# bdaiinstitute/vlfm

Hardware: AMD Instinct MI355X
Metric: env-steps/s (VLM+value-map update), 640x480 RGB-D (higher is better)
Workload: dtype f16 ViT-g (f32 accumulate) + f32 Q-Former (split-f16, 22-bit); f32 confidence + f64 value maps; 1 GPU; configs[1] step x resident envs: BLIP-2 ITC + ValueMap+ObstacleMap+sort_waypoints; envs_per_gpu=256, global_envs=256, map=1000x1000 @ 20 px/m, parallelism=env-sharded x1, tuned_gemms=True, vit_gemm=hip:fc1, attention=hip

## Files before the change

### include/vlfm_amd.h

```cpp
#ifndef VLFM_AMD_H
#define VLFM_AMD_H

#include <stddef.h>
#include <stdint.h>

#ifdef __cplusplus
extern "C" {
#endif

typedef enum {
    VLFM_OK = 0,
    VLFM_ERR_INVALID = -1,
    VLFM_ERR_OUTSIDE_MAP = -2,
    VLFM_ERR_INDEX = -3,
    VLFM_ERR_HIP = -4,
    VLFM_ERR_CAPACITY = -5
} vlfm_status;

enum { VLFM_FUSE_DEFAULT = 0, VLFM_FUSE_REPLACE = 1, VLFM_FUSE_EQUAL_WEIGHTING = 2 };

const char* vlfm_last_error(void);
int vlfm_abi_version(void);

int vlfm_profile_enable(int on);
// ... 134 lines not shown
                        const int32_t* d_text_index, int n_prompts, float* d_out, void* stream);

int vlfm_layernorm_bias_f16(const void* d_x, const float* d_channel_bias, const void* d_gamma, const void* d_beta,
                            void* d_y, int rows, int dim, float eps, void* stream);

int vlfm_vit_attention_f16(const void* d_qkv, void* d_out, int batch, int tokens, int heads, int head_dim, float scale,
                           void* stream);

int vlfm_gemm_f16_nt(const void* d_x, const void* d_w, const void* d_bias, void* d_c, int m, int n, int k, int epilogue,
                     void* stream);

int vlfm_gemm_f16_pair_f32_nt(const void* d_x, const void* d_w_pair, const void* d_bias_f32, void* d_out, int m, int n_out, int k,
                              void* stream);

int vlfm_qformer_cross_attention_f32(const void* d_q, const void* d_kv_blocks, void* d_out, int batch, int tokens, int queries,
                                     int heads, int k_block0, int v_block0, int m_total, float scale, void* stream);

int vlfm_gemm_f16_tile_order(int m, int n, int group_m, int* out, int capacity_pairs);
int vlfm_gemm_f16_work_items(int m, int n, int grid, int* out, int capacity_pairs);

int vlfm_split_f32_to_f16_pair(const float* d_src, void* d_hi, void* d_lo, long long count, int* d_overflow, void* stream);
int vlfm_gemm_f32_nt(const float* d_x, const float* d_w, const float* d_bias, const float* d_residual, float* d_c, int m, int n,
                     int k, int activation, int precision, const void* d_w_hi, const void* d_w_lo, int* d_overflow, void* stream);


int vlfm_layernorm_rows_f32(const float* d_x, const float* d_gamma, const float* d_beta, float* d_out, int batch, int height,
                            int width, int channels, int window, float eps, void* stream);
int vlfm_window_reverse_add_f32(float* d_x, const float* d_windows, int batch, int height, int width, int channels, int window,
                                void* stream);
int vlfm_dwconv3x3_nhwc_f32(const float* d_x, const float* d_w9c, const float* d_bias, float* d_out, int batch, int height, int width,
                            int channels, void* stream);
int vlfm_window_attention_f32(const float* d_qkv, const float* d_bias_t, float* d_out, long long windows, int tokens, int heads,
                              float scale, void* stream);
int vlfm_layernorm_rows_shifted_f32(const float* d_x, const float* d_gamma, const float* d_beta, float* d_out, int batch, int height,
                                    int width, int channels, int window, float eps, int shift, int pad_zero, void* stream);
int vlfm_window_reverse_add_shifted_f32(float* d_x, const float* d_windows, int batch, int height, int width, int channels, int window,
                                        int shift, void* stream);
int vlfm_window_attention_masked_f32(const float* d_qkv, const float* d_bias_t, const float* d_mask_t, int windows_per_image, float* d_out,
                                     long long windows, int tokens, int heads, float scale, void* stream);

int vlfm_maxpool2x2_nhwc_f16(const void* d_x, void* d_out, int batch, int height, int width, int channels, void* stream);
int vlfm_conv_nhwc_tile(int pixels, int cin, int cout, int ksize, int* tile_pixels, int* tile_channels);
int vlfm_conv_nhwc_f16(const void* d_x, const void* d_w, const void* d_bias, void* d_out, const void* d_zero, int batch,
                       int height, int width, int cin, int cout, int ksize, int stride, int x_pix_stride,
                       int out_pix_stride, int act, void* stream);

// ... 188 lines not shown
```

### vlfm_amd/_lib.py

```python
from __future__ import annotations

import ctypes
import os
import subprocess
from typing import Optional

_HERE = os.path.dirname(os.path.abspath(__file__))
LIB_PATH = os.path.join(_HERE, "libvlfm_amd.so")
SOURCES = ["value_map.hip", "depth_ingest.hip", "depth_holes.hip", "obstacle_map.hip", "vlm_ops.hip", "vit_attention.hip", "qformer_attention.hip", "detect_ops.hip", "object_cloud.hip", "gemm_f16.hip", "gemm_f32.hip", "conv_nhwc.hip", "sam_ops.hip", "map_render.hip", "jpeg_codec.hip", "jpeg_entropy.hip", "jpeg_decode.hip", "world_render.hip", "host.cpp"]

VLFM_OK = 0
VLFM_ERR_INVALID = -1
VLFM_ERR_OUTSIDE_MAP = -2
VLFM_ERR_INDEX = -3
VLFM_ERR_HIP = -4
VLFM_ERR_CAPACITY = -5

FUSION_TYPES = {"default": 0, "replace": 1, "equal_weighting": 2}


class VmPose(ctypes.Structure):
    _fields_ = [("inv_affine", ctypes.c_double * 6), ("row0", ctypes.c_int32), ("col0", ctypes.c_int32),
                ("env", ctypes.c_int32), ("reserved", ctypes.c_int32)]

# ... 80 lines not shown
        L.vlfm_profile_read.argtypes = [ctypes.c_char_p, ctypes.POINTER(cd), ctypes.POINTER(ci)]
        L.vlfm_value_map_pose_params.argtypes = [vp, vp, vp, ci, ci, ci, ci, vp, ctypes.POINTER(ci)]
        L.vlfm_cone_template_host.argtypes = [cd, cd, ci, cd, vp, ci, vp, ci, ctypes.POINTER(ci)]
        L.vlfm_tan_table_host.argtypes = [cd, ci, vp]
        L.vlfm_disc_rows_host.argtypes = [ci, vp]
        L.vlfm_cone_template_build.argtypes = [vp, vp, ci, ci, vp, vp, vp]
        L.vlfm_depth_ingest_batched.argtypes = [vp, ci, ci, ci, vp, vp, vp, ci, ci, vp, vp, vp, vp, vp]
        L.vlfm_selftest_div_exact.argtypes = [vp, ci, cd, vp, vp]
        L.vlfm_hole_scratch_bytes.argtypes = [ci, ci, ci, ci, ci]
        L.vlfm_hole_scratch_bytes.restype = ctypes.c_size_t
        L.vlfm_fill_small_holes_batched.argtypes = [vp, vp, ci, ci, ci, cd, vp, ctypes.c_size_t, ci, ci, vp, vp, vp, vp,
                                                    ci, vp, vp]
        L.vlfm_depth_scatter_holes_batched.argtypes = [vp, ci, ci, ci, vp, vp, vp, vp, ci, ci, vp, vp, vp]
        L.vlfm_fill_small_holes_rig_batched.argtypes = [vp, vp, ci, ci, ci, cd, vp, ctypes.c_size_t, ci, ci, vp, vp, vp, vp,
                                                        ci, vp, vp, ci, vp]
        L.vlfm_depth_scatter_holes_rig_batched.argtypes = [vp, ci, ci, ci, vp, vp, vp, vp, ci, ci, vp, vp, vp, vp]
        L.vlfm_layernorm_bias_f16.argtypes = [vp, vp, vp, vp, vp, ci, ci, ctypes.c_float, vp]
        L.vlfm_vit_attention_f16.argtypes = [vp, vp, ci, ci, ci, ci, ctypes.c_float, vp]
        L.vlfm_gemm_f16_nt.argtypes = [vp, vp, vp, vp, ci, ci, ci, ci, vp]
        L.vlfm_gemm_f16_pair_f32_nt.argtypes = [vp, vp, vp, vp, ci, ci, ci, vp]
        L.vlfm_qformer_cross_attention_f32.argtypes = [vp, vp, vp, ci, ci, ci, ci, ci, ci, ci, ctypes.c_float, vp]
        L.vlfm_gemm_f32_nt.argtypes = [vp, vp, vp, vp, vp, ci, ci, ci, ci, ci, vp, vp, vp, vp]
        L.vlfm_split_f32_to_f16_pair.argtypes = [vp, vp, vp, ctypes.c_longlong, vp, vp]
        L.vlfm_layernorm_rows_f32.argtypes = [vp, vp, vp, vp, ci, ci, ci, ci, ci, ctypes.c_float, vp]
        L.vlfm_window_reverse_add_f32.argtypes = [vp, vp, ci, ci, ci, ci, ci, vp]
        L.vlfm_dwconv3x3_nhwc_f32.argtypes = [vp, vp, vp, vp, ci, ci, ci, ci, vp]
        L.vlfm_window_attention_f32.argtypes = [vp, vp, vp, ctypes.c_longlong, ci, ci, ctypes.c_float, vp]
        L.vlfm_layernorm_rows_shifted_f32.argtypes = [vp, vp, vp, vp, ci, ci, ci, ci, ci, ctypes.c_float, ci, ci, vp]
        L.vlfm_window_reverse_add_shifted_f32.argtypes = [vp, vp, ci, ci, ci, ci, ci, ci, vp]
        L.vlfm_window_attention_masked_f32.argtypes = [vp, vp, vp, ci, vp, ctypes.c_longlong, ci, ci, ctypes.c_float, vp]
        L.vlfm_maxpool2x2_nhwc_f16.argtypes = [vp, vp, ci, ci, ci, ci, vp]
        L.vlfm_conv_nhwc_tile.argtypes = [ci, ci, ci, ci, ctypes.POINTER(ci), ctypes.POINTER(ci)]
        L.vlfm_conv_nhwc_f16.argtypes = [vp, vp, vp, vp, vp, ci, ci, ci, ci, ci, ci, ci, ci, ci, ci, vp]
        L.vlfm_value_map_update_fused_batched.argtypes = [vp, ci, vp, vp, vp, ci, vp, vp, ci, vp, vp, ci, ci, ci, cd, cd,
                                                          ci, ci, vp, vp, vp, vp, vp]
        L.vlfm_value_map_update_rig_batched.argtypes = [vp, ci, vp, vp, vp, ci, ci, ci, vp, vp, vp, ci, ci, ci, ci, ci, vp, vp,
                                                        vp, vp]
        L.vlfm_value_map_sort_waypoints_batched.argtypes = [vp, ci, ci, vp, ci, ci, vp, ci, vp, vp]
        L.vlfm_resample_coeffs_host.argtypes = [ci, ci, vp, vp, ci, ctypes.POINTER(ci)]
        L.vlfm_resample_coeffs_filter_host.argtypes = [ci, ci, ci, vp, vp, ci, ctypes.POINTER(ci)]
        L.vlfm_preprocess_sam_batched.argtypes = [vp, ci, ci, ci, ci, ci, vp, vp, ci, vp, vp, ci, vp, vp, ci, vp, vp, vp]
        L.vlfm_preprocess_rgb_batched.argtypes = [vp, ci, ci, ci, ci, vp, vp, ci, vp, vp, ci, vp, vp, vp, vp, ci, ci, vp]
        L.vlfm_itc_head_batched.argtypes = [vp, ci, ci, ci, vp, vp, vp]
        L.vlfm_itc_head_multi.argtypes = [vp, ci, ci, ci, vp, ci, vp, ci, vp, vp]
        cf = ctypes.c_float
        L.vlfm_resize_area_tab_host.argtypes = [ci, ci, vp, vp, vp, ci]
# ... 111 lines not shown
```

### vlfm_amd/csrc/gemm_f32.hip

```cpp
#include <hip/hip_runtime.h>
#include <stdint.h>
#include <stdlib.h>

#include "../../include/vlfm_amd.h"
#include "profile.h"
#include "status.h"

namespace vlfm {
namespace g32 {

typedef float floatx4 __attribute__((ext_vector_type(4)));
typedef float floatx16 __attribute__((ext_vector_type(16)));
typedef _Float16 half8 __attribute__((ext_vector_type(8)));
typedef _Float16 half4 __attribute__((ext_vector_type(4)));

constexpr int TB = 128;
constexpr int TK = 32;
constexpr int ROWB = TK * 4;
constexpr int OPER = TB * ROWB;
constexpr int BUF = 2 * OPER;
constexpr int EPI_ROW = 272;
constexpr int EPI_WAVE = 64 * EPI_ROW;
constexpr int LDS_EXACT = 4 * EPI_WAVE > 2 * BUF ? 4 * EPI_WAVE : 2 * BUF;

enum { ACT_NONE = 0, ACT_RELU = 1, ACT_GELU = 2 };

struct Args {
    const float* x;
    const float* w;
    const float* bias;
    const float* residual;
    float* c;
    int M, N, K;
    int tiles_m, tiles_n;
    int* overflow;
    const _Float16* w_hi;
    const _Float16* w_lo;
};

__device__ inline float gelu_erf(float v) {
    const float u = fabsf(v);
    float q = 2.834908400e-06f;
    q = fmaf(q, u, -3.937762449e-05f);
    q = fmaf(q, u, 1.861798810e-04f);
    q = fmaf(q, u, 1.369373058e-04f);
    q = fmaf(q, u, -7.063421421e-03f);
    q = fmaf(q, u, 5.249617994e-02f);
    q = fmaf(q, u, 4.592081904e-01f);
    q = fmaf(q, u, 1.151105165e+00f);
    const float e = __builtin_amdgcn_exp2f(-(q * u));
    return fmaf(-0.5f * u, e, fmaxf(v, 0.0f));
}

using lds_ptr = __attribute__((address_space(3))) unsigned char*;
using gbl_ptr = const __attribute__((address_space(1))) unsigned char*;

__device__ inline void tile_of_block(const Args& a, int& tm, int& tn) {
    const int nwg = a.tiles_m * a.tiles_n;
    int bid = blockIdx.x;
    const int q = nwg >> 3, r = nwg & 7, xcd = bid & 7, idx = bid >> 3;
    bid = (xcd < r ? xcd * (q + 1) : r * (q + 1) + (xcd - r) * q) + idx;
    tm = bid / a.tiles_n;
    tn = bid - tm * a.tiles_n;
}

__device__ inline void stage_tile(const Args& a, lds_ptr lds, int buf, int n0, int m0, int k0, int wave, int lane) {
    const int sub = lane >> 3, p = lane & 7;
#pragma unroll
    for (int j = 0; j < 4; j++) {
        const int chunk = wave * 4 + j;
        const int r = chunk * 8 + sub;
        const int s = p ^ ((r >> 1) & 7);
        const int rn = min(n0 + r, a.N - 1), rm = min(m0 + r, a.M - 1);
        const float* gw = a.w + (size_t)rn * a.K + k0 + s * 4;
        const float* gx = a.x + (size_t)rm * a.K + k0 + s * 4;
        const int dst = __builtin_amdgcn_readfirstlane(buf + chunk * 1024);
        __builtin_amdgcn_global_load_lds((gbl_ptr)gw, lds + dst, 16, 0, 0);
        __builtin_amdgcn_global_load_lds((gbl_ptr)gx, lds + dst + OPER, 16, 0, 0);
    }
}

template <bool SPLIT>
__device__ inline void store_tile(const Args& a, unsigned char* smem, const floatx16 (&acc)[2][2], const floatx16 (&cross)[2][2],
                                  int act, int wave, int wn, int wm, int lane, int m0, int n0) {
    unsigned char* stg = smem + wave * EPI_WAVE;
    const int c32 = lane & 31, h4 = (lane >> 5) * 4;
    floatx4 bias4[2][4];
#pragma unroll
    for (int i = 0; i < 2; i++)
#pragma unroll
        for (int g = 0; g < 4; g++) {
            floatx4 b = {0.f, 0.f, 0.f, 0.f};
            if (a.bias) {
                const int n = n0 + wn * 64 + i * 32 + g * 8 + h4;
                if (n + 4 <= a.N && ((uintptr_t)a.bias & 15) == 0) b = *reinterpret_cast<const floatx4*>(a.bias + n);
                else
                    for (int e = 0; e < 4; e++) b[e] = n + e < a.N ? a.bias[n + e] : 0.f;
            }
            bias4[i][g] = b;
        }
#pragma unroll
    for (int i = 0; i < 2; i++)
#pragma unroll
        for (int g = 0; g < 4; g++) {
            const int nl = i * 32 + g * 8 + h4;
            const floatx4 b = bias4[i][g];
#pragma unroll
// ... 10 lines not shown
                }
                *reinterpret_cast<floatx4*>(stg + (j * 32 + c32) * EPI_ROW + nl * 4) = v;
            }
        }
    __builtin_amdgcn_s_waitcnt(0xC07F);
    const int rsub = lane >> 4, chunk = lane & 15;
    const bool vec = (a.N & 3) == 0;
    const int n = n0 + wn * 64 + chunk * 4;
    const bool fast = vec && n + 4 <= a.N;
    floatx4 r[16], v[16];
#pragma unroll
    for (int it = 0; it < 16; it++) {
        const int m = m0 + wm * 64 + it * 4 + rsub;
        r[it] = floatx4{0.f, 0.f, 0.f, 0.f};
        if (a.residual && fast && m < a.M) r[it] = *reinterpret_cast<const floatx4*>(a.residual + (size_t)m * a.N + n);
    }
#pragma unroll
    for (int it = 0; it < 16; it++) v[it] = *reinterpret_cast<const floatx4*>(stg + (it * 4 + rsub) * EPI_ROW + chunk * 16);
#pragma unroll
    for (int it = 0; it < 16; it++) {
        const int m = m0 + wm * 64 + it * 4 + rsub;
        if (m >= a.M || n >= a.N) continue;
        const size_t at = (size_t)m * a.N + n;
        if (fast) {
            *reinterpret_cast<floatx4*>(a.c + at) = v[it] + r[it];
        } else {
            for (int e = 0; e < 4 && n + e < a.N; e++) a.c[at + e] = v[it][e] + (a.residual ? a.residual[at + e] : 0.f);
        }
    }
}

__global__ __launch_bounds__(256, 2) void gemm_f32_exact_kernel(Args a, int act) {
    extern __shared__ __attribute__((aligned(16))) unsigned char smem[];
    lds_ptr lds = (lds_ptr)smem;
    const int tid = threadIdx.x, lane = tid & 63;
    const int wave = __builtin_amdgcn_readfirstlane(tid >> 6);
    const int wn = wave >> 1, wm = wave & 1;
    int tm, tn;
    tile_of_block(a, tm, tn);
    const int m0 = tm * TB, n0 = tn * TB;
    const int NT = a.K / TK;

    floatx16 acc[2][2];
#pragma unroll
    for (int i = 0; i < 2; i++)
#pragma unroll
        for (int j = 0; j < 2; j++)
// ... 15 lines not shown
            floatx4 fa[2], fb[2];
#pragma unroll
            for (int i = 0; i < 2; i++) {
                const int R = wn * 64 + i * 32 + r32;
                fa[i] = *reinterpret_cast<const floatx4*>(smem + cur + R * ROWB + ((s ^ ((R >> 1) & 7)) << 4));
            }
#pragma unroll
            for (int j = 0; j < 2; j++) {
                const int R = wm * 64 + j * 32 + r32;
                fb[j] = *reinterpret_cast<const floatx4*>(smem + cur + OPER + R * ROWB + ((s ^ ((R >> 1) & 7)) << 4));
            }
#pragma unroll
            for (int q = 0; q < 4; q++)
#pragma unroll
                for (int i = 0; i < 2; i++)
#pragma unroll
                    for (int j = 0; j < 2; j++)
                        acc[i][j] = __builtin_amdgcn_mfma_f32_32x32x2f32(fa[i][q], fb[j][q], acc[i][j], 0, 0, 0);
        }
        __builtin_amdgcn_s_waitcnt(0x0F70);
        __builtin_amdgcn_s_barrier();
        asm volatile("" ::: "memory");
    }
    store_tile<false>(a, smem, acc, acc, act, wave, wn, wm, lane, m0, n0);
}

constexpr int SROWB = TK * 2;
constexpr int SOPER = TB * SROWB;
constexpr int SBUF = 4 * SOPER;

__device__ inline int sslot(int row, int slot) { return (slot ^ ((row >> 2) & 3)) << 4; }

__device__ inline void split4(const floatx4 v, half4& hi, half4& lo, bool& over) {
#pragma unroll
    for (int e = 0; e < 4; e++) {
        const float a = v[e];
        over |= !(fabsf(a) < 65504.0f);
        const _Float16 hh = (_Float16)a;
        hi[e] = hh;
        lo[e] = (_Float16)((a - (float)hh) * 2048.0f);
    }
}

template <int NI>
struct SplitGeom {
    static constexpr int TN = 64 * NI;
    static constexpr int WOPER = TN * SROWB;
    static constexpr int XO = 0, WO = 2 * SOPER;
    static constexpr int BUF = 2 * SOPER + 2 * WOPER;
    static constexpr int LDS = 4 * EPI_WAVE > 2 * BUF ? 4 * EPI_WAVE : 2 * BUF;
};

template <int NI>
__device__ __forceinline__ void gemm_f32_split_body(const Args& a, int act) {
    using G = SplitGeom<NI>;
    extern __shared__ __attribute__((aligned(16))) unsigned char smem[];
    lds_ptr lds = (lds_ptr)smem;
    const int tid = threadIdx.x, lane = tid & 63;
    const int wave = __builtin_amdgcn_readfirstlane(tid >> 6);
    const int wn = wave >> 1, wm = wave & 1;
    int tm, tn;
    tile_of_block(a, tm, tn);
    const int m0 = tm * TB, n0 = tn * G::TN;
    const int NT = a.K / TK;

// ... 72 lines not shown
                xhi[j] = *reinterpret_cast<const half8*>(smem + o);
                xlo[j] = *reinterpret_cast<const half8*>(smem + o + SOPER);
            }
#pragma unroll
            for (int i = 0; i < NI; i++)
#pragma unroll
                for (int j = 0; j < 2; j++) {
                    acc[i][j] = __builtin_amdgcn_mfma_f32_32x32x16_f16(whi[i], xhi[j], acc[i][j], 0, 0, 0);
                    crs[i][j] = __builtin_amdgcn_mfma_f32_32x32x16_f16(whi[i], xlo[j], crs[i][j], 0, 0, 0);
                    crs[i][j] = __builtin_amdgcn_mfma_f32_32x32x16_f16(wlo[i], xhi[j], crs[i][j], 0, 0, 0);
                }
        }
        if (t + 1 < NT) put_x(cur ^ G::BUF);
        __builtin_amdgcn_s_waitcnt(0x0F70);
        __builtin_amdgcn_s_waitcnt(0xC07F);
        __builtin_amdgcn_s_barrier();
        asm volatile("" ::: "memory");
    }
    if (over && a.overflow) atomicOr(a.overflow, 1);
#pragma unroll
    for (int half = 0; half < NI / 2; half++)
        store_tile<true>(a, smem, reinterpret_cast<const floatx16(&)[2][2]>(acc[2 * half]),
                         reinterpret_cast<const floatx16(&)[2][2]>(crs[2 * half]), act, wave, 0, wm, lane, m0,
                         n0 + wn * 32 * NI + half * 64);
}

__global__ __launch_bounds__(256, 2) void gemm_f32_split_kernel(Args a, int act) { gemm_f32_split_body<2>(a, act); }

__global__ void split_f32_kernel(const float* __restrict__ src, _Float16* __restrict__ hi, _Float16* __restrict__ lo, long long n,
                                 int* overflow) {
    const long long i = (long long)blockIdx.x * blockDim.x + threadIdx.x;
    if (i >= n) return;
    const float a = src[i];
    if (!(fabsf(a) < 65504.0f) && overflow) atomicOr(overflow, 1);
    const _Float16 hh = (_Float16)a;
    hi[i] = hh;
    lo[i] = (_Float16)((a - (float)hh) * 2048.0f);
}

}
}

using namespace vlfm;
using namespace vlfm::g32;

extern "C" int vlfm_split_f32_to_f16_pair(const float* d_src, void* d_hi, void* d_lo, long long count, int* d_overflow, void* stream) {
    if (count == 0) return VLFM_OK;
    if (!d_src || !d_hi || !d_lo || count < 0) return fail(VLFM_ERR_INVALID, "split_f32_to_f16_pair: bad argument");
    const long long blocks = (count + 255) / 256;
    VLFM_KLAUNCH(split_f32_kernel, dim3((unsigned)blocks), dim3(256), 0, (hipStream_t)stream, d_src, (_Float16*)d_hi, (_Float16*)d_lo,
                 count, d_overflow);
    return check_launch("split_f32_kernel");
}

extern "C" int vlfm_gemm_f32_nt(const float* d_x, const float* d_w, const float* d_bias, const float* d_residual, float* d_c, int m,
                                int n, int k, int activation, int precision, const void* d_w_hi, const void* d_w_lo,
                                int* d_overflow, void* stream) {
    if (m == 0 || n == 0) return VLFM_OK;
    if (!d_x || !d_w || !d_c || m < 0 || n < 0 || k <= 0 || (k % TK) != 0 || activation < 0 || activation > 2 || precision < 0 ||
        precision > 1)
        return fail(VLFM_ERR_INVALID, "gemm_f32_nt: K must be a multiple of 32, activation 0..2, precision 0..1");
    if (((uintptr_t)d_x | (uintptr_t)d_w | (uintptr_t)d_c | (uintptr_t)d_residual | (uintptr_t)d_w_hi | (uintptr_t)d_w_lo) & 15)
        return fail(VLFM_ERR_INVALID, "gemm_f32_nt: X, W, C, residual and the split weights must be 16-byte aligned");
    if (precision == 1 && (!d_w_hi || !d_w_lo || !d_overflow))
        return fail(VLFM_ERR_INVALID, "gemm_f32_nt: the split form needs the pre-split weights and the overflow flag");
    Args a;
    a.x = d_x; a.w = d_w; a.bias = d_bias; a.residual = d_residual; a.c = d_c;
    a.M = m; a.N = n; a.K = k;
    a.tiles_m = (m + TB - 1) / TB; a.tiles_n = (n + TB - 1) / TB;
    a.overflow = d_overflow; a.w_hi = (const _Float16*)d_w_hi; a.w_lo = (const _Float16*)d_w_lo;
    if ((long long)a.tiles_m * a.tiles_n > 0x7fffffffLL) return fail(VLFM_ERR_CAPACITY, "gemm_f32_nt: too many tiles");
    const dim3 grid(a.tiles_m * a.tiles_n), block(256);
    static LdsOptIn opt_exact, opt_split;
    if (precision == 0) {
        if (LDS_EXACT > 64 * 1024 && !opt_exact.ensure(reinterpret_cast<const void*>(gemm_f32_exact_kernel), LDS_EXACT))
            return fail(VLFM_ERR_HIP, "gemm_f32_nt: cannot opt in to the LDS size");
        VLFM_TIMED("gemm_f32_exact_kernel", stream);
        VLFM_KLAUNCH(gemm_f32_exact_kernel, grid, block, LDS_EXACT, (hipStream_t)stream, a, activation);
        return check_launch("gemm_f32_exact_kernel");
    }
    if (SplitGeom<2>::LDS > 64 * 1024 && !opt_split.ensure(reinterpret_cast<const void*>(gemm_f32_split_kernel), SplitGeom<2>::LDS))
        return fail(VLFM_ERR_HIP, "gemm_f32_nt: cannot opt in to the LDS size");
    VLFM_TIMED("gemm_f32_split_kernel", stream);
    VLFM_KLAUNCH(gemm_f32_split_kernel, grid, block, SplitGeom<2>::LDS, (hipStream_t)stream, a, activation);
    return check_launch("gemm_f32_split_kernel");
}
```

### vlfm_amd/csrc/host.cpp

```cpp
#include <cmath>
#include <cstdint>
#include <cstring>
#include <mutex>
#include <string>

#include "../../include/vlfm_amd.h"
#include "status.h"

namespace vlfm {
static thread_local std::string g_last_error;
void set_last_error(const char* msg) { g_last_error = msg ? msg : ""; }
}

extern "C" const char* vlfm_last_error(void) { return vlfm::g_last_error.c_str(); }
extern "C" int vlfm_abi_version(void) { return 17; }

namespace {

const double kPi = 3.141592653589793238462643383279502884;

inline long round_half_even(double v) { return std::lrint(v); }

float sin_deg_table(int deg) {
    static float tab[451];
    static std::once_flag once;
    std::call_once(once, [] {
        for (int i = 0; i <= 450; i++) tab[i] = (float)(std::round(std::sin(i * kPi / 180.0) * 1e7) / 1e7);
    });
    return tab[deg];
}

}

extern "C" int vlfm_value_map_pose_params(const double* h_tf, const double* h_yaw, const int32_t* h_env, int n,
                                          int map_size, int pixels_per_meter, int template_size,
                                          vlfm_vm_pose* h_out, int* bad_index) {
    if (!h_tf || !h_out || n < 0 || map_size <= 0 || template_size <= 0)
        return vlfm::fail(VLFM_ERR_INVALID, "value_map_pose_params: bad argument");
// ... 255 lines not shown
```

### vlfm_amd/vlm/blip2itm.py

```python
from __future__ import annotations

import hashlib
import math
import os
import re
from dataclasses import dataclass
from typing import Dict, List, Optional, Sequence, Tuple

import numpy as np
import torch
import torch.nn as nn
import torch.nn.functional as F


@dataclass
class Blip2ITCConfig:
    image_size: int = 224
    patch_size: int = 14
    v_hidden: int = 1408
    v_layers: int = 39
    v_heads: int = 16
    v_mlp: int = 6144
    v_ln_eps: float = 1e-6
    q_hidden: int = 768
# ... 139 lines not shown
    w1 = w.half()
    r = (w - w1.float()) * 2048.0
    w2 = r.half()
    return w1, w2, ((r - w2.float()) * 2048.0).half()


KV_SPLIT_PIECES = 2


def _split_gemm(x16: torch.Tensor, pieces, bias: torch.Tensor, n_pieces: Optional[int] = None) -> torch.Tensor:
    w1t, w2t, w3t = pieces
    if (KV_SPLIT_PIECES if n_pieces is None else n_pieces) >= 3:
        o = torch.addmm(bias, x16, w3t, alpha=2.0 ** -22, out_dtype=torch.float32)
        torch.addmm(o, x16, w2t, alpha=2.0 ** -11, out_dtype=torch.float32, out=o)
    else:
        o = torch.addmm(bias, x16, w2t, alpha=2.0 ** -11, out_dtype=torch.float32)
    torch.addmm(o, x16, w1t, out_dtype=torch.float32, out=o)
    return o


QFORMER_SPLIT_MIN_ROWS = 2048


def _qlinear(x: torch.Tensor, lin_w: torch.Tensor, lin_b, act=None, residual=None) -> torch.Tensor:
    from . import ops

    if (x.is_cuda and x.dtype == torch.float32 and lin_w.dtype == torch.float32 and not torch.is_grad_enabled()
            and x.numel() // x.shape[-1] >= QFORMER_SPLIT_MIN_ROWS and ops.linear_f32_supported(x, lin_w)):
        return ops.linear_f32(x, lin_w, lin_b, act=act, residual=residual, precision="split", owner="blip2")
    y = F.linear(x, lin_w, lin_b)
    if act == "gelu":
        y = F.gelu(y)
    return y if residual is None else y + residual


class _BertAttention(nn.Module):
    def __init__(self, hidden: int, kv_hidden: int, heads: int, eps: float):
        super().__init__()
        self.heads = heads
        self.query = nn.Linear(hidden, hidden)
        self.key = nn.Linear(kv_hidden, hidden)
        self.value = nn.Linear(kv_hidden, hidden)
        self.dense = nn.Linear(hidden, hidden)
        self.LayerNorm = nn.LayerNorm(hidden, eps=eps)
        self._kv_split = None
        self._qkv_fused = None

    def _project_kv_f16(self, kv16: torch.Tensor) -> Tuple[torch.Tensor, torch.Tensor]:
        if self._kv_split is None or self._kv_split[0].device != kv16.device:
            w1, w2, w3 = _exact_split3(torch.cat([self.key.weight, self.value.weight]))
            bias = torch.cat([self.key.bias, self.value.bias]).detach().float()
            self._kv_split = (w1.t(), w2.t(), w3.t(), bias)
        o = _split_gemm(kv16.reshape(-1, kv16.shape[-1]), self._kv_split[:3], self._kv_split[3])
        o = o.view(*kv16.shape[:-1], -1)
        hid = self.key.out_features
        return o[..., :hid], o[..., hid:]

    def forward(self, x: torch.Tensor, kv: Optional[torch.Tensor] = None, mask: Optional[torch.Tensor] = None,
                kv_proj: Optional[Tuple[torch.Tensor, torch.Tensor]] = None, kv_blocks=None) -> torch.Tensor:
        b, n, d = x.shape
        h = self.heads
        if kv_blocks is not None:
            from . import ops

            blocks, tokens, k_block0, v_block0 = kv_blocks
            q = _qlinear(x, self.query.weight, self.query.bias).contiguous()
            a = ops.qformer_cross_attention(q, blocks, tokens, h, k_block0, v_block0, (d // h) ** -0.5)
            return self.LayerNorm(_qlinear(a, self.dense.weight, self.dense.bias, residual=x))
        if kv_proj is not None:
            q = _qlinear(x, self.query.weight, self.query.bias).view(b, n, h, d // h).transpose(1, 2)
            k = kv_proj[0].reshape(b, -1, h, d // h).transpose(1, 2)
            v = kv_proj[1].reshape(b, -1, h, d // h).transpose(1, 2)
        elif kv is None and x.is_cuda and not self.training:
            if self._qkv_fused is None or self._qkv_fused[0].device != x.device or self._qkv_fused[0].dtype != x.dtype:
                self._qkv_fused = (torch.cat([self.query.weight, self.key.weight, self.value.weight]).detach(),
                                   torch.cat([self.query.bias, self.key.bias, self.value.bias]).detach())
            qkv = _qlinear(x, *self._qkv_fused).view(b, n, 3, h, d // h).permute(2, 0, 3, 1, 4)
            q, k, v = qkv[0], qkv[1], qkv[2]
        else:
            q = self.query(x).view(b, n, h, d // h).transpose(1, 2)
            if kv is not None and kv.dtype == torch.float16 and kv.is_cuda and self.key.weight.dtype == torch.float32:
                k, v = self._project_kv_f16(kv)
                src_len = kv.shape[1]
            else:
                src = x if kv is None else kv.to(x.dtype)
                k, v, src_len = self.key(src), self.value(src), src.shape[1]
            k = k.reshape(b, src_len, h, d // h).transpose(1, 2)
            v = v.reshape(b, src_len, h, d // h).transpose(1, 2)
        a = F.scaled_dot_product_attention(q, k, v, attn_mask=mask)
        return self.LayerNorm(_qlinear(a.transpose(1, 2).reshape(b, n, d), self.dense.weight, self.dense.bias,
                                       residual=x))


class _BertFFN(nn.Module):
    def __init__(self, hidden: int, inter: int, eps: float):
        super().__init__()
        self.up = nn.Linear(hidden, inter)
        self.down = nn.Linear(inter, hidden)
        self.LayerNorm = nn.LayerNorm(hidden, eps=eps)

    def forward(self, x: torch.Tensor) -> torch.Tensor:
        hid = _qlinear(x, self.up.weight, self.up.bias, act="gelu")
        return self.LayerNorm(_qlinear(hid, self.down.weight, self.down.bias, residual=x))


class _QFormerLayer(nn.Module):
    def __init__(self, c: Blip2ITCConfig, idx: int):
        super().__init__()
        self.attention = _BertAttention(c.q_hidden, c.q_hidden, c.q_heads, c.q_ln_eps)
        self.crossattention = (_BertAttention(c.q_hidden, c.v_hidden, c.q_heads, c.q_ln_eps)
                               if idx % c.cross_attention_frequency == 0 else None)
        self.ffn_text = _BertFFN(c.q_hidden, c.q_mlp, c.q_ln_eps)
        self.ffn_query = _BertFFN(c.q_hidden, c.q_mlp, c.q_ln_eps)


class Blip2ITCModel(nn.Module):

    def __init__(self, cfg: Blip2ITCConfig):
        super().__init__()
        c = self.cfg = cfg
        n_patches = (c.image_size // c.patch_size) ** 2
        self.class_embedding = nn.Parameter(torch.zeros(1, 1, c.v_hidden))
        self.position_embedding = nn.Parameter(torch.zeros(1, n_patches + 1, c.v_hidden))
        self.patch_embedding = nn.Conv2d(3, c.v_hidden, c.patch_size, c.patch_size)
        self.blocks = nn.ModuleList([_VitBlock(c) for _ in range(c.v_layers)])
        self.post_layernorm = nn.LayerNorm(c.v_hidden, eps=c.v_ln_eps)
        self.query_tokens = nn.Parameter(torch.zeros(1, c.num_query_tokens, c.q_hidden))
        self.word_embeddings = nn.Embedding(c.vocab_size, c.q_hidden)
        self.position_embeddings = nn.Embedding(c.max_position_embeddings, c.q_hidden)
        self.q_layernorm = nn.LayerNorm(c.q_hidden, eps=c.q_ln_eps)
        self.q_layers = nn.ModuleList([_QFormerLayer(c, i) for i in range(c.q_layers)])
        self.vision_projection = nn.Linear(c.q_hidden, c.proj_dim)
        self.text_projection = nn.Linear(c.q_hidden, c.proj_dim)
        self.deferred_bias = True
        self._deferred_c: Optional[torch.Tensor] = None
        self.split_kv = True
        self.split_kv_min_rows = 32 * 257
        self._kv_all = None
        self.fused_cross_kv = True
        self._kv_pair = None

    def init_random(self, seed: int = 0) -> "Blip2ITCModel":
        dev = self.query_tokens.device
        g = torch.Generator(device=dev).manual_seed(seed)
        with torch.no_grad():
            for p in self.parameters():
                if p.dim() > 1:
                    p.copy_(torch.randn(p.shape, generator=g, device=dev) * 0.02)
                else:
                    p.zero_()
            for m in self.modules():
                if isinstance(m, nn.LayerNorm):
                    m.weight.fill_(1.0)
        self.weights_changed()
        return self

    def weights_changed(self) -> None:
        self._deferred_c = None
        self._kv_all = None
        self._kv_pair = None
        for layer in self.q_layers:
            layer.attention._qkv_fused = None
            if layer.crossattention is not None:
# ... 157 lines not shown
        return self.post_layernorm(x)

    def _deferred_constants(self) -> torch.Tensor:
        if self._deferred_c is None or self._deferred_c.device != self.post_layernorm.weight.device:
            rows, run = [], torch.zeros(self.cfg.v_hidden, dtype=torch.float32, device=self.post_layernorm.weight.device)
            for blk in self.blocks:
                rows.append(run.clone())
                run = run + blk.projection.bias.detach().float()
                rows.append(run.clone())
                run = run + blk.fc2.bias.detach().float()
            rows.append(run.clone())
            self._deferred_c = torch.stack(rows).contiguous()
        return self._deferred_c

    def query_features(self, image_tokens: torch.Tensor) -> torch.Tensor:
        split_ok = (self.split_kv and image_tokens.dtype == torch.float16 and image_tokens.is_cuda
                    and image_tokens.shape[0] * image_tokens.shape[1] >= self.split_kv_min_rows)
        enc = image_tokens if split_ok else image_tokens.to(self.q_layernorm.weight.dtype)
        h = self.q_layernorm(self.query_tokens).expand(enc.shape[0], -1, -1)
        fused = split_ok and self._fused_cross_ok(enc)
        blocks = self._project_all_kv_blocks(enc) if fused else None
        proj = self._project_all_kv(enc) if split_ok and not fused else None
        hid, at = self.cfg.q_hidden, 0
        for layer in self.q_layers:
            h = layer.attention(h)
            if layer.crossattention is not None:
                if blocks is not None:
                    h = layer.crossattention(h, kv_blocks=(blocks, enc.shape[1], at // 64, (at + hid) // 64))
                    at += 2 * hid
                elif proj is not None:
                    h = layer.crossattention(h, kv_proj=(proj[..., at:at + hid], proj[..., at + hid:at + 2 * hid]))
                    at += 2 * hid
                else:
                    h = layer.crossattention(h, kv=enc)
            h = layer.ffn_query(h)
        return h

    def _fused_cross_ok(self, tokens16: torch.Tensor) -> bool:
        from . import ops

        c = self.cfg
        return (self.fused_cross_kv and KV_SPLIT_PIECES == 2 and not torch.is_grad_enabled()
                and self.q_layernorm.weight.dtype == torch.float32
                and c.q_hidden % c.q_heads == 0 and c.q_hidden // c.q_heads == ops.QFORMER_ATTENTION_HEAD
                and c.num_query_tokens <= ops.QFORMER_ATTENTION_MAX_QUERIES
                and 1 <= tokens16.shape[1] <= ops.QFORMER_ATTENTION_MAX_TOKENS and c.v_hidden % 64 == 0
                and tokens16.shape[0] * tokens16.shape[1] * c.v_hidden * 2 < (1 << 32))

    def _kv_all_pieces(self, device):
        if self._kv_all is None or self._kv_all[0].device != device:
            cross = [l.crossattention for l in self.q_layers if l.crossattention is not None]
            w = torch.cat([torch.cat([c.key.weight, c.value.weight]) for c in cross])
            bias = torch.cat([torch.cat([c.key.bias, c.value.bias]) for c in cross]).detach().float()
            w1, w2, w3 = _exact_split3(w)
            self._kv_all = (w1.t(), w2.t(), w3.t(), bias)
            self._kv_pair = None
        return self._kv_all

# ... 315 lines not shown
```

### vlfm_amd/vlm/ops.py

```python
from __future__ import annotations

import ctypes
from typing import Dict, Optional, Tuple

import numpy as np
import torch

from .. import _lib

CLIP_MEAN = (0.48145466, 0.4578275, 0.40821073)
CLIP_STD = (0.26862954, 0.26130258, 0.27577711)
_DTYPE_CODE = {torch.float32: 0, torch.float16: 1, torch.bfloat16: 2}
_coeff_cache: Dict[Tuple[str, int, int], Tuple[torch.Tensor, torch.Tensor, int]] = {}


def _stream() -> int:
    return torch._C._cuda_getCurrentRawStream(torch._C._cuda_getDevice())


def resample_coeffs(in_size: int, out_size: int, bilinear: bool = False) -> Tuple[np.ndarray, np.ndarray, int]:
    bounds = np.zeros((out_size, 2), np.int32)
    cap = out_size * (2 * int(np.ceil(2.0 * max(1.0, in_size / out_size))) + 1)
    kk = np.zeros(cap, np.int32)
    ks = ctypes.c_int(0)
# ... 381 lines not shown
    w = weight if weight.is_contiguous() else weight.contiguous()
    M = x2.shape[0]
    if out is None:
        out = torch.empty((M, N), dtype=torch.float32, device=x.device)
    res = None
    if residual is not None:
        res = residual.reshape(M, N)
        if not res.is_contiguous() or res.data_ptr() % 16:
            res = res.contiguous()
    b = None
    if bias is not None:
        b = bias if bias.is_contiguous() else bias.contiguous()
    prec = GEMM_F32_PRECISION[precision]
    hi = lo = None
    if prec == 1:
        hi, lo = split_weight(w, owner)
    _lib.check(_lib.lib().vlfm_gemm_f32_nt(x2.data_ptr(), w.data_ptr(), b.data_ptr() if b is not None else None,
                                           res.data_ptr() if res is not None else None, out.data_ptr(), M, N, K, _ACT32[act], prec,
                                           hi.data_ptr() if hi is not None else None, lo.data_ptr() if lo is not None else None,
                                           gemm_f32_overflow_flag(x.device, owner).data_ptr(), _stream()), "gemm_f32_nt")
    return out.view(*lead, N)


_tuned_gemms_state = None


def use_tuned_gemms() -> bool:
    global _tuned_gemms_state
    if _tuned_gemms_state is None:
        import os

        path = os.path.join(os.path.dirname(os.path.dirname(os.path.abspath(__file__))), "tunableop_results.csv")
        ok = False
        if os.environ.get("VLFM_TUNED_GEMMS", "1") != "0" and os.path.exists(path) and torch.cuda.is_available():
            try:
                import torch.cuda.tunable as tunable

                import tempfile

                tunable.enable(True)
                tunable.tuning_enable(False)
                tunable.set_filename(os.path.join(tempfile.gettempdir(), f"vlfm_amd_tunableop_{os.getpid()}.csv"))
                ok = bool(tunable.read_file(path))
            except Exception as exc:
                import warnings

# ... 5 lines not shown
```

Before: 1767 env-steps/s.

## Feed Q-Former split GEMMs pre-split f16 activation planes and emit FFN hidden as planes

New measurement: 1770 env-steps/s (median of 2 runs). Within noise of the previous version (+0.2%).

```diff
diff --git a/include/vlfm_amd.h b/include/vlfm_amd.h
--- a/include/vlfm_amd.h
+++ b/include/vlfm_amd.h
@@ -180,6 +180,9 @@
 int vlfm_split_f32_to_f16_pair(const float* d_src, void* d_hi, void* d_lo, long long count, int* d_overflow, void* stream);
 int vlfm_gemm_f32_nt(const float* d_x, const float* d_w, const float* d_bias, const float* d_residual, float* d_c, int m, int n,
                      int k, int activation, int precision, const void* d_w_hi, const void* d_w_lo, int* d_overflow, void* stream);
+int vlfm_gemm_f32_planes_nt(const void* d_x_hi, const void* d_x_lo, const void* d_w_hi, const void* d_w_lo, const float* d_bias,
+                            const float* d_residual, float* d_c, void* d_c_hi, void* d_c_lo, int m, int n, int k, int activation,
+                            int* d_overflow, void* stream);
 
 
 int vlfm_layernorm_rows_f32(const float* d_x, const float* d_gamma, const float* d_beta, float* d_out, int batch, int height,
diff --git a/vlfm_amd/_lib.py b/vlfm_amd/_lib.py
--- a/vlfm_amd/_lib.py
+++ b/vlfm_amd/_lib.py
@@ -126,6 +126,7 @@
         L.vlfm_qformer_cross_attention_f32.argtypes = [vp, vp, vp, ci, ci, ci, ci, ci, ci, ci, ctypes.c_float, vp]
         L.vlfm_gemm_f32_nt.argtypes = [vp, vp, vp, vp, vp, ci, ci, ci, ci, ci, vp, vp, vp, vp]
         L.vlfm_split_f32_to_f16_pair.argtypes = [vp, vp, vp, ctypes.c_longlong, vp, vp]
+        L.vlfm_gemm_f32_planes_nt.argtypes = [vp, vp, vp, vp, vp, vp, vp, vp, vp, ci, ci, ci, ci, vp, vp]
         L.vlfm_layernorm_rows_f32.argtypes = [vp, vp, vp, vp, ci, ci, ci, ci, ci, ctypes.c_float, vp]
         L.vlfm_window_reverse_add_f32.argtypes = [vp, vp, ci, ci, ci, ci, ci, vp]
         L.vlfm_dwconv3x3_nhwc_f32.argtypes = [vp, vp, vp, vp, ci, ci, ci, ci, vp]
diff --git a/vlfm_amd/csrc/gemm_f32.hip b/vlfm_amd/csrc/gemm_f32.hip
--- a/vlfm_amd/csrc/gemm_f32.hip
+++ b/vlfm_amd/csrc/gemm_f32.hip
@@ -36,6 +36,10 @@
     int* overflow;
     const _Float16* w_hi;
     const _Float16* w_lo;
+    const _Float16* x_hi;
+    const _Float16* x_lo;
+    _Float16* c_hi;
+    _Float16* c_lo;
 };
 
 __device__ inline float gelu_erf(float v) {
@@ -80,9 +84,20 @@
     }
 }
 
-template <bool SPLIT>
+__device__ inline void split4(const floatx4 v, half4& hi, half4& lo, bool& over) {
+#pragma unroll
+    for (int e = 0; e < 4; e++) {
+        const float a = v[e];
+        over |= !(fabsf(a) < 65504.0f);
+        const _Float16 hh = (_Float16)a;
+        hi[e] = hh;
+        lo[e] = (_Float16)((a - (float)hh) * 2048.0f);
+    }
+}
+
+template <bool SPLIT, bool PLANES = false>
 __device__ inline void store_tile(const Args& a, unsigned char* smem, const floatx16 (&acc)[2][2], const floatx16 (&cross)[2][2],
-                                  int act, int wave, int wn, int wm, int lane, int m0, int n0) {
+                                  int act, int wave, int wn, int wm, int lane, int m0, int n0, bool& over) {
     unsigned char* stg = smem + wave * EPI_WAVE;
     const int c32 = lane & 31, h4 = (lane >> 5) * 4;
     floatx4 bias4[2][4];
@@ -139,7 +154,19 @@
         const int m = m0 + wm * 64 + it * 4 + rsub;
         if (m >= a.M || n >= a.N) continue;
         const size_t at = (size_t)m * a.N + n;
-        if (fast) {
+        if (PLANES) {
+            floatx4 o = v[it] + r[it];
+            if (!fast)
+                for (int e = 0; e < 4; e++) o[e] = n + e < a.N ? v[it][e] + (a.residual ? a.residual[at + e] : 0.f) : 0.f;
+            half4 hi, lo;
+            split4(o, hi, lo, over);
+            if (fast) {
+                *reinterpret_cast<half4*>(a.c_hi + at) = hi;
+                *reinterpret_cast<half4*>(a.c_lo + at) = lo;
+            } else {
+                for (int e = 0; e < 4 && n + e < a.N; e++) { a.c_hi[at + e] = hi[e]; a.c_lo[at + e] = lo[e]; }
+            }
+        } else if (fast) {
             *reinterpret_cast<floatx4*>(a.c + at) = v[it] + r[it];
         } else {
             for (int e = 0; e < 4 && n + e < a.N; e++) a.c[at + e] = v[it][e] + (a.residual ? a.residual[at + e] : 0.f);
@@ -201,7 +228,8 @@
         __builtin_amdgcn_s_barrier();
         asm volatile("" ::: "memory");
     }
-    store_tile<false>(a, smem, acc, acc, act, wave, wn, wm, lane, m0, n0);
+    bool unused = false;
+    store_tile<false>(a, smem, acc, acc, act, wave, wn, wm, lane, m0, n0, unused);
 }
 
 constexpr int SROWB = TK * 2;
@@ -209,17 +237,6 @@
 constexpr int SBUF = 4 * SOPER;
 
 __device__ inline int sslot(int row, int slot) { return (slot ^ ((row >> 2) & 3)) << 4; }
-
-__device__ inline void split4(const floatx4 v, half4& hi, half4& lo, bool& over) {
-#pragma unroll
-    for (int e = 0; e < 4; e++) {
-        const float a = v[e];
-        over |= !(fabsf(a) < 65504.0f);
-        const _Float16 hh = (_Float16)a;
-        hi[e] = hh;
-        lo[e] = (_Float16)((a - (float)hh) * 2048.0f);
-    }
-}
 
 template <int NI>
 struct SplitGeom {
@@ -338,20 +355,116 @@
     for (int half = 0; half < NI / 2; half++)
         store_tile<true>(a, smem, reinterpret_cast<const floatx16(&)[2][2]>(acc[2 * half]),
                          reinterpret_cast<const floatx16(&)[2][2]>(crs[2 * half]), act, wave, 0, wm, lane, m0,
-                         n0 + wn * 32 * NI + half * 64);
+                         n0 + wn * 32 * NI + half * 64, over);
 }
 
 __global__ __launch_bounds__(256, 2) void gemm_f32_split_kernel(Args a, int act) { gemm_f32_split_body<2>(a, act); }
 
+template <bool PLANES_OUT>
+__global__ __launch_bounds__(256, 2) void gemm_f32_split_planes_kernel(Args a, int act) {
+    using G = SplitGeom<2>;
+    extern __shared__ __attribute__((aligned(16))) unsigned char smem[];
+    lds_ptr lds = (lds_ptr)smem;
+    const int tid = threadIdx.x, lane = tid & 63;
+    const int wave = __builtin_amdgcn_readfirstlane(tid >> 6);
+    const int wn = wave >> 1, wm = wave & 1;
+    int tm, tn;
+    tile_of_block(a, tm, tn);
+    const int m0 = tm * TB, n0 = tn * G::TN;
+    const int NT = a.K / TK;
+
+    floatx16 acc[2][2], crs[2][2];
+#pragma unroll
+    for (int i = 0; i < 2; i++)
+#pragma unroll
+        for (int j = 0; j < 2; j++)
+#pragma unroll
+            for (int e = 0; e < 16; e++) { acc[i][j][e] = 0.f; crs[i][j][e] = 0.f; }
+
+    const int sub = lane >> 2, p = lane & 3;
+    size_t gw[2], gx[2];
+#pragma unroll
+    for (int j = 0; j < 2; j++) {
+        const int r = (wave * 2 + j) * 16 + sub;
+        const int s = p ^ ((r >> 2) & 3);
+        gw[j] = (size_t)min(n0 + r, a.N - 1) * a.K + s * 8;
+        gx[j] = (size_t)min(m0 + r, a.M - 1) * a.K + s * 8;
+    }
+    auto stage = [&](int buf, int k0) {
+#pragma unroll
+        for (int j = 0; j < 2; j++) {
+            const int dst = __builtin_amdgcn_readfirstlane(buf + (wave * 2 + j) * 1024);
+            __builtin_amdgcn_global_load_lds((gbl_ptr)(a.w_hi + gw[j] + k0), lds + dst + G::WO, 16, 0, 0);
+            __builtin_amdgcn_global_load_lds((gbl_ptr)(a.w_lo + gw[j] + k0), lds + dst + G::WO + G::WOPER, 16, 0, 0);
+            __builtin_amdgcn_global_load_lds((gbl_ptr)(a.x_hi + gx[j] + k0), lds + dst + G::XO, 16, 0, 0);
+            __builtin_amdgcn_global_load_lds((gbl_ptr)(a.x_lo + gx[j] + k0), lds + dst + G::XO + SOPER, 16, 0, 0);
+        }
+    };
+
+    stage(0, 0);
+    __builtin_amdgcn_s_waitcnt(0x0F70);
+    __builtin_amdgcn_s_barrier();
+    asm volatile("" ::: "memory");
+
+    const int r32 = lane & 31, h = lane >> 5;
+    for (int t = 0; t < NT; t++) {
+        const int cur = (t & 1) * G::BUF;
+        if (t + 1 < NT) stage(cur ^ G::BUF, (t + 1) * TK);
+#pragma unroll
+        for (int kk = 0; kk < 2; kk++) {
+            const int s = kk * 2 + h;
+            half8 whi[2], wlo[2], xhi[2], xlo[2];
+#pragma unroll
+            for (int i = 0; i < 2; i++) {
+                const int R = wn * 64 + i * 32 + r32, o = cur + G::WO + R * SROWB + sslot(R, s);
+                whi[i] = *reinterpret_cast<const half8*>(smem + o);
+                wlo[i] = *reinterpret_cast<const half8*>(smem + o + G::WOPER);
+            }
+#pragma unroll
+            for (int j = 0; j < 2; j++) {
+                const int R = wm * 64 + j * 32 + r32, o = cur + G::XO + R * SROWB + sslot(R, s);
+                xhi[j] = *reinterpret_cast<const half8*>(smem + o);
+                xlo[j] = *reinterpret_cast<const half8*>(smem + o + SOPER);
+            }
+#pragma unroll
+            for (int i = 0; i < 2; i++)
+#pragma unroll
+                for (int j = 0; j < 2; j++) {
+                    acc[i][j] = __builtin_amdgcn_mfma_f32_32x32x16_f16(whi[i], xhi[j], acc[i][j], 0, 0, 0);
+                    crs[i][j] = __builtin_amdgcn_mfma_f32_32x32x16_f16(whi[i], xlo[j], crs[i][j], 0, 0, 0);
+                    crs[i][j] = __builtin_amdgcn_mfma_f32_32x32x16_f16(wlo[i], xhi[j], crs[i][j], 0, 0, 0);
+                }
+        }
+        __builtin_amdgcn_s_waitcnt(0x0F70);
+        __builtin_amdgcn_s_waitcnt(0xC07F);
+        __builtin_amdgcn_s_barrier();
+        asm volatile("" ::: "memory");
+    }
+    bool over = false;
+    store_tile<true, PLANES_OUT>(a, smem, acc, crs, act, wave, 0, wm, lane, m0, n0 + wn * 64, over);
+    if (PLANES_OUT && over && a.overflow) atomicOr(a.overflow, 1);
+}
+
 __global__ void split_f32_kernel(const float* __restrict__ src, _Float16* __restrict__ hi, _Float16* __restrict__ lo, long long n,
-                                 int* overflow) {
-    const long long i = (long long)blockIdx.x * blockDim.x + threadIdx.x;
-    if (i >= n) return;
-    const float a = src[i];
-    if (!(fabsf(a) < 65504.0f) && overflow) atomicOr(overflow, 1);
-    const _Float16 hh = (_Float16)a;
-    hi[i] = hh;
-    lo[i] = (_Float16)((a - (float)hh) * 2048.0f);
+                                 int* overflow, int vec4) {
+    const long long t = (long long)blockIdx.x * blockDim.x + threadIdx.x;
+    bool over = false;
+    if (vec4 && 4 * t + 4 <= n) {
+        half4 h4, l4;
+        split4(*reinterpret_cast<const floatx4*>(src + 4 * t), h4, l4, over);
+        *reinterpret_cast<half4*>(hi + 4 * t) = h4;
+        *reinterpret_cast<half4*>(lo + 4 * t) = l4;
+    } else {
+        const long long i0 = vec4 ? 4 * t : t, i1 = vec4 ? n : min(t + 1, n);
+        for (long long i = i0; i < i1; i++) {
+            const float a = src[i];
+            over |= !(fabsf(a) < 65504.0f);
+            const _Float16 hh = (_Float16)a;
+            hi[i] = hh;
+            lo[i] = (_Float16)((a - (float)hh) * 2048.0f);
+        }
+    }
+    if (over && overflow) atomicOr(overflow, 1);
 }
 
 }
@@ -363,10 +476,49 @@
 extern "C" int vlfm_split_f32_to_f16_pair(const float* d_src, void* d_hi, void* d_lo, long long count, int* d_overflow, void* stream) {
     if (count == 0) return VLFM_OK;
     if (!d_src || !d_hi || !d_lo || count < 0) return fail(VLFM_ERR_INVALID, "split_f32_to_f16_pair: bad argument");
-    const long long blocks = (count + 255) / 256;
+    const int vec4 = (((uintptr_t)d_src & 15) | ((uintptr_t)d_hi & 7) | ((uintptr_t)d_lo & 7)) == 0;
+    const long long threads = vec4 ? (count + 3) / 4 : count, blocks = (threads + 255) / 256;
+    if (blocks > 0x7fffffffLL) return fail(VLFM_ERR_CAPACITY, "split_f32_to_f16_pair: too many elements");
+    VLFM_TIMED("split_f32_kernel", stream);
     VLFM_KLAUNCH(split_f32_kernel, dim3((unsigned)blocks), dim3(256), 0, (hipStream_t)stream, d_src, (_Float16*)d_hi, (_Float16*)d_lo,
-                 count, d_overflow);
+                 count, d_overflow, vec4);
     return check_launch("split_f32_kernel");
+}
+
+extern "C" int vlfm_gemm_f32_planes_nt(const void* d_x_hi, const void* d_x_lo, const void* d_w_hi, const void* d_w_lo,
+                                       const float* d_bias, const float* d_residual, float* d_c, void* d_c_hi, void* d_c_lo, int m,
+                                       int n, int k, int activation, int* d_overflow, void* stream) {
+    if (m == 0 || n == 0) return VLFM_OK;
+    const bool planes_out = d_c == nullptr;
+    if (!d_x_hi || !d_x_lo || !d_w_hi || !d_w_lo || m < 0 || n < 0 || k <= 0 || (k % TK) != 0 || activation < 0 || activation > 2 ||
+        (planes_out ? (!d_c_hi || !d_c_lo || !d_overflow) : (d_c_hi || d_c_lo)))
+        return fail(VLFM_ERR_INVALID, "gemm_f32_planes_nt: needs all four operand planes, K a multiple of 32, activation 0..2 and "
+                                      "either C or both result planes with the overflow flag");
+    if (((uintptr_t)d_x_hi | (uintptr_t)d_x_lo | (uintptr_t)d_w_hi | (uintptr_t)d_w_lo | (uintptr_t)d_c | (uintptr_t)d_c_hi |
+         (uintptr_t)d_c_lo | (uintptr_t)d_residual) & 15)
+        return fail(VLFM_ERR_INVALID, "gemm_f32_planes_nt: the planes, C and residual must be 16-byte aligned");
+    Args a;
+    a.x = nullptr; a.w = nullptr; a.bias = d_bias; a.residual = d_residual; a.c = d_c;
+    a.M = m; a.N = n; a.K = k;
+    a.tiles_m = (m + TB - 1) / TB; a.tiles_n = (n + TB - 1) / TB;
+    a.overflow = d_overflow; a.w_hi = (const _Float16*)d_w_hi; a.w_lo = (const _Float16*)d_w_lo;
+    a.x_hi = (const _Float16*)d_x_hi; a.x_lo = (const _Float16*)d_x_lo; a.c_hi = (_Float16*)d_c_hi; a.c_lo = (_Float16*)d_c_lo;
+    if ((long long)a.tiles_m * a.tiles_n > 0x7fffffffLL) return fail(VLFM_ERR_CAPACITY, "gemm_f32_planes_nt: too many tiles");
+    const dim3 grid(a.tiles_m * a.tiles_n), block(256);
+    static LdsOptIn opt_f32, opt_planes;
+    constexpr int LDS = SplitGeom<2>::LDS;
+    if (planes_out) {
+        if (LDS > 64 * 1024 && !opt_planes.ensure(reinterpret_cast<const void*>(gemm_f32_split_planes_kernel<true>), LDS))
+            return fail(VLFM_ERR_HIP, "gemm_f32_planes_nt: cannot opt in to the LDS size");
+        VLFM_TIMED("gemm_f32_split_planes_kernel", stream);
+        VLFM_KLAUNCH(gemm_f32_split_planes_kernel<true>, grid, block, LDS, (hipStream_t)stream, a, activation);
+    } else {
+        if (LDS > 64 * 1024 && !opt_f32.ensure(reinterpret_cast<const void*>(gemm_f32_split_planes_kernel<false>), LDS))
+            return fail(VLFM_ERR_HIP, "gemm_f32_planes_nt: cannot opt in to the LDS size");
+        VLFM_TIMED("gemm_f32_split_planes_kernel", stream);
+        VLFM_KLAUNCH(gemm_f32_split_planes_kernel<false>, grid, block, LDS, (hipStream_t)stream, a, activation);
+    }
+    return check_launch("gemm_f32_split_planes_kernel");
 }
 
 extern "C" int vlfm_gemm_f32_nt(const float* d_x, const float* d_w, const float* d_bias, const float* d_residual, float* d_c, int m,
@@ -385,6 +537,7 @@
     a.M = m; a.N = n; a.K = k;
     a.tiles_m = (m + TB - 1) / TB; a.tiles_n = (n + TB - 1) / TB;
     a.overflow = d_overflow; a.w_hi = (const _Float16*)d_w_hi; a.w_lo = (const _Float16*)d_w_lo;
+    a.x_hi = a.x_lo = nullptr; a.c_hi = a.c_lo = nullptr;
     if ((long long)a.tiles_m * a.tiles_n > 0x7fffffffLL) return fail(VLFM_ERR_CAPACITY, "gemm_f32_nt: too many tiles");
     const dim3 grid(a.tiles_m * a.tiles_n), block(256);
     static LdsOptIn opt_exact, opt_split;
diff --git a/vlfm_amd/csrc/host.cpp b/vlfm_amd/csrc/host.cpp
--- a/vlfm_amd/csrc/host.cpp
+++ b/vlfm_amd/csrc/host.cpp
@@ -13,7 +13,7 @@
 }
 
 extern "C" const char* vlfm_last_error(void) { return vlfm::g_last_error.c_str(); }
-extern "C" int vlfm_abi_version(void) { return 17; }
+extern "C" int vlfm_abi_version(void) { return 18; }
 
 namespace {
 
diff --git a/vlfm_amd/vlm/blip2itm.py b/vlfm_amd/vlm/blip2itm.py
--- a/vlfm_amd/vlm/blip2itm.py
+++ b/vlfm_amd/vlm/blip2itm.py
@@ -185,11 +185,23 @@
 QFORMER_SPLIT_MIN_ROWS = 2048
 
 
-def _qlinear(x: torch.Tensor, lin_w: torch.Tensor, lin_b, act=None, residual=None) -> torch.Tensor:
+QFORMER_PLANES_SHAPES = frozenset({(2304, 768), (3072, 768), (768, 3072)})
+
+
+def _qlinear_split_ok(x: torch.Tensor, lin_w: torch.Tensor) -> bool:
     from . import ops
 
-    if (x.is_cuda and x.dtype == torch.float32 and lin_w.dtype == torch.float32 and not torch.is_grad_enabled()
-            and x.numel() // x.shape[-1] >= QFORMER_SPLIT_MIN_ROWS and ops.linear_f32_supported(x, lin_w)):
+    return (x.is_cuda and x.dtype == torch.float32 and lin_w.dtype == torch.float32 and not torch.is_grad_enabled()
+            and x.numel() // x.shape[-1] >= QFORMER_SPLIT_MIN_ROWS and ops.linear_f32_supported(x, lin_w))
+
+
+def _qlinear(x: torch.Tensor, lin_w: torch.Tensor, lin_b, act=None, residual=None, planes: bool = False) -> torch.Tensor:
+    from . import ops
+
+    if _qlinear_split_ok(x, lin_w):
+        if planes and tuple(lin_w.shape) in QFORMER_PLANES_SHAPES:
+            xp = ops.split_f32(x if x.is_contiguous() else x.contiguous(), owner="blip2")
+            return ops.linear_f32_planes(xp, lin_w, lin_b, act=act, residual=residual, owner="blip2")
         return ops.linear_f32(x, lin_w, lin_b, act=act, residual=residual, precision="split", owner="blip2")
     y = F.linear(x, lin_w, lin_b)
     if act == "gelu":
@@ -220,25 +232,25 @@
         return o[..., :hid], o[..., hid:]
 
     def forward(self, x: torch.Tensor, kv: Optional[torch.Tensor] = None, mask: Optional[torch.Tensor] = None,
-                kv_proj: Optional[Tuple[torch.Tensor, torch.Tensor]] = None, kv_blocks=None) -> torch.Tensor:
+                kv_proj: Optional[Tuple[torch.Tensor, torch.Tensor]] = None, kv_blocks=None, planes: bool = False) -> torch.Tensor:
         b, n, d = x.shape
         h = self.heads
         if kv_blocks is not None:
             from . import ops
 
             blocks, tokens, k_block0, v_block0 = kv_blocks
-            q = _qlinear(x, self.query.weight, self.query.bias).contiguous()
+            q = _qlinear(x, self.query.weight, self.query.bias, planes=planes).contiguous()
             a = ops.qformer_cross_attention(q, blocks, tokens, h, k_block0, v_block0, (d // h) ** -0.5)
-            return self.LayerNorm(_qlinear(a, self.dense.weight, self.dense.bias, residual=x))
+            return self.LayerNorm(_qlinear(a, self.dense.weight, self.dense.bias, residual=x, planes=planes))
         if kv_proj is not None:
-            q = _qlinear(x, self.query.weight, self.query.bias).view(b, n, h, d // h).transpose(1, 2)
+            q = _qlinear(x, self.query.weight, self.query.bias, planes=planes).view(b, n, h, d // h).transpose(1, 2)
             k = kv_proj[0].reshape(b, -1, h, d // h).transpose(1, 2)
             v = kv_proj[1].reshape(b, -1, h, d // h).transpose(1, 2)
         elif kv is None and x.is_cuda and not self.training:
             if self._qkv_fused is None or self._qkv_fused[0].device != x.device or self._qkv_fused[0].dtype != x.dtype:
                 self._qkv_fused = (torch.cat([self.query.weight, self.key.weight, self.value.weight]).detach(),
                                    torch.cat([self.query.bias, self.key.bias, self.value.bias]).detach())
-            qkv = _qlinear(x, *self._qkv_fused).view(b, n, 3, h, d // h).permute(2, 0, 3, 1, 4)
+            qkv = _qlinear(x, *self._qkv_fused, planes=planes).view(b, n, 3, h, d // h).permute(2, 0, 3, 1, 4)
             q, k, v = qkv[0], qkv[1], qkv[2]
         else:
             q = self.query(x).view(b, n, h, d // h).transpose(1, 2)
@@ -252,7 +264,7 @@
             v = v.reshape(b, src_len, h, d // h).transpose(1, 2)
         a = F.scaled_dot_product_attention(q, k, v, attn_mask=mask)
         return self.LayerNorm(_qlinear(a.transpose(1, 2).reshape(b, n, d), self.dense.weight, self.dense.bias,
-                                       residual=x))
+                                       residual=x, planes=planes))
 
 
 class _BertFFN(nn.Module):
@@ -262,9 +274,17 @@
         self.down = nn.Linear(inter, hidden)
         self.LayerNorm = nn.LayerNorm(hidden, eps=eps)
 
-    def forward(self, x: torch.Tensor) -> torch.Tensor:
-        hid = _qlinear(x, self.up.weight, self.up.bias, act="gelu")
-        return self.LayerNorm(_qlinear(hid, self.down.weight, self.down.bias, residual=x))
+    def forward(self, x: torch.Tensor, planes: bool = False) -> torch.Tensor:
+        up, down = self.up, self.down
+        if (planes and tuple(up.weight.shape) in QFORMER_PLANES_SHAPES and tuple(down.weight.shape) in QFORMER_PLANES_SHAPES
+                and _qlinear_split_ok(x, up.weight) and down.weight.dtype == torch.float32 and down.weight.shape[1] % 32 == 0):
+            from . import ops
+
+            xp = ops.split_f32(x if x.is_contiguous() else x.contiguous(), owner="blip2")
+            hid = ops.linear_f32_planes(xp, up.weight, up.bias, act="gelu", out_planes=True, owner="blip2")
+            return self.LayerNorm(ops.linear_f32_planes(hid, down.weight, down.bias, residual=x, owner="blip2"))
+        hid = _qlinear(x, up.weight, up.bias, act="gelu", planes=planes)
+        return self.LayerNorm(_qlinear(hid, down.weight, down.bias, residual=x, planes=planes))
 
 
 class _QFormerLayer(nn.Module):
@@ -302,6 +322,7 @@
         self._kv_all = None
         self.fused_cross_kv = True
         self._kv_pair = None
+        self.split_planes = True
 
     def init_random(self, seed: int = 0) -> "Blip2ITCModel":
         dev = self.query_tokens.device
@@ -505,18 +526,20 @@
         blocks = self._project_all_kv_blocks(enc) if fused else None
         proj = self._project_all_kv(enc) if split_ok and not fused else None
         hid, at = self.cfg.q_hidden, 0
+        planes = bool(self.split_planes)
         for layer in self.q_layers:
-            h = layer.attention(h)
+            h = layer.attention(h, planes=planes)
             if layer.crossattention is not None:
                 if blocks is not None:
-                    h = layer.crossattention(h, kv_blocks=(blocks, enc.shape[1], at // 64, (at + hid) // 64))
+                    h = layer.crossattention(h, kv_blocks=(blocks, enc.shape[1], at // 64, (at + hid) // 64), planes=planes)
                     at += 2 * hid
                 elif proj is not None:
-                    h = layer.crossattention(h, kv_proj=(proj[..., at:at + hid], proj[..., at + hid:at + 2 * hid]))
+                    h = layer.crossattention(h, kv_proj=(proj[..., at:at + hid], proj[..., at + hid:at + 2 * hid]),
+                                             planes=planes)
                     at += 2 * hid
                 else:
-                    h = layer.crossattention(h, kv=enc)
-            h = layer.ffn_query(h)
+                    h = layer.crossattention(h, kv=enc, planes=planes)
+            h = layer.ffn_query(h, planes=planes)
         return h
 
     def _fused_cross_ok(self, tokens16: torch.Tensor) -> bool:
diff --git a/vlfm_amd/vlm/ops.py b/vlfm_amd/vlm/ops.py
--- a/vlfm_amd/vlm/ops.py
+++ b/vlfm_amd/vlm/ops.py
@@ -427,6 +427,56 @@
     return out.view(*lead, N)
 
 
+def split_f32(x: torch.Tensor, owner: str = "", out=None) -> Tuple[torch.Tensor, torch.Tensor]:
+    assert x.is_cuda and x.dtype == torch.float32 and x.is_contiguous()
+    hi, lo = out if out is not None else (torch.empty(x.shape, dtype=torch.float16, device=x.device),
+                                          torch.empty(x.shape, dtype=torch.float16, device=x.device))
+    assert hi.shape == x.shape == lo.shape and hi.dtype == lo.dtype == torch.float16 and hi.is_contiguous() and lo.is_contiguous()
+    _lib.check(_lib.lib().vlfm_split_f32_to_f16_pair(x.data_ptr(), hi.data_ptr(), lo.data_ptr(), x.numel(),
+                                                     gemm_f32_overflow_flag(x.device, owner).data_ptr(), _stream()), "split_f32")
+    return hi, lo
+
+
+def linear_f32_planes(x_planes: Tuple[torch.Tensor, torch.Tensor], weight: torch.Tensor, bias=None, act=None, residual=None,
+                      out=None, out_planes=False, owner: str = ""):
+    x_hi, x_lo = x_planes
+    K, N = weight.shape[1], weight.shape[0]
+    assert x_hi.is_cuda and x_hi.dtype == x_lo.dtype == torch.float16 and x_hi.shape == x_lo.shape and x_hi.shape[-1] == K
+    assert x_hi.is_contiguous() and x_lo.is_contiguous() and weight.dtype == torch.float32
+    lead = x_hi.shape[:-1]
+    M = x_hi.numel() // K
+    w = weight if weight.is_contiguous() else weight.contiguous()
+    w_hi, w_lo = split_weight(w, owner)
+    res = None
+    if residual is not None:
+        res = residual.reshape(M, N)
+        if not res.is_contiguous() or res.data_ptr() % 16:
+            res = res.contiguous()
+    b = None
+    if bias is not None:
+        b = bias if bias.is_contiguous() else bias.contiguous()
+    c = c_hi = c_lo = None
+    if out_planes:
+        c_hi, c_lo = out if out is not None else (torch.empty((M, N), dtype=torch.float16, device=x_hi.device),
+                                                  torch.empty((M, N), dtype=torch.float16, device=x_hi.device))
+        assert c_hi.dtype == c_lo.dtype == torch.float16 and c_hi.numel() == c_lo.numel() == M * N
+        assert c_hi.is_contiguous() and c_lo.is_contiguous()
+    else:
+        c = out if out is not None else torch.empty((M, N), dtype=torch.float32, device=x_hi.device)
+        assert c.dtype == torch.float32 and c.numel() == M * N and c.is_contiguous()
+    _lib.check(_lib.lib().vlfm_gemm_f32_planes_nt(x_hi.data_ptr(), x_lo.data_ptr(), w_hi.data_ptr(), w_lo.data_ptr(),
+                                                  b.data_ptr() if b is not None else None,
+                                                  res.data_ptr() if res is not None else None,
+                                                  c.data_ptr() if c is not None else None,
+                                                  c_hi.data_ptr() if c_hi is not None else None,
+                                                  c_lo.data_ptr() if c_lo is not None else None, M, N, K, _ACT32[act],
+                                                  gemm_f32_overflow_flag(x_hi.device, owner).data_ptr(), _stream()),
+               "gemm_f32_planes_nt")
+    if out_planes:
+        return c_hi.view(*lead, N), c_lo.view(*lead, N)
+    return c.view(*lead, N)
+
+
 _tuned_gemms_state = None
 
 
```
